# heracles-ec/heracles

Measured on AMD Instinct MI355X. Metric: map->Cl pairs/sec + mixing-matrix build sec, nside=4096 lmax=6144, higher is better.
Workload: dtype f64

## Files before the change

### heracles_amd/csrc/hx_analysis.hip

```cpp
#include <algorithm>
#include <cmath>
#include <cstdlib>
#include <cstring>

#include "hx_sht_common.h"

namespace hx {
using namespace hxfft;

constexpr int HALF_F = 1;
template <int SPIN>
struct LegCfg {
    static constexpr int NW = SPIN == 0 ? 16 : 8;
    static constexpr int NT = SPIN == 0 ? 1 : 2;
    static constexpr int NOP = SPIN == 0 ? 1 : 2;
    static constexpr int NPAR = (SPIN == 2 && HALF_F) ? 1 : 2;
};
int analysis_f_rows(int spin) { return spin == 0 ? LegCfg<0>::NPAR * LegCfg<0>::NOP : LegCfg<2>::NPAR * LegCfg<2>::NOP; }

struct LegParams {
    PlanDev P;
    const LegTask *__restrict__ tasks;
    const double *__restrict__ F;
    double *__restrict__ partial;
    int m0, ms;
    long long row0;
    int ng;
    int ncol;
    int pcol;
    const MTasks *__restrict__ of_m;
    const long long *__restrict__ arow;
    long long arow0;
    int add_all;
};

template <int SPIN>
__global__ __launch_bounds__(256) void k_fourier_combine(PlanDev P, const double2 *__restrict__ Y, int ncomp, int ng,
                                                         int ncol, int m0, int ms, const double *__restrict__ rw,
                                                         const LegTask *__restrict__ tasks, const MTasks *__restrict__ of_m,
                                                         double *__restrict__ F, int tile0)
{
    constexpr int NOP = LegCfg<SPIN>::NOP;
    __shared__ RingAtM ring_at_m[32];
    const int m = m0 + blockIdx.x * ms;
    const int ty = (int)blockIdx.y + tile0;
    const MTasks mt = of_m[m];
    if (mt.count == 0 || ty < tasks[mt.first].rb0) return;
    if (threadIdx.x < 32) ring_at_m[threadIdx.x] = ring_at_m_of(P, ty * 32 + threadIdx.x, m, rw);
    __syncthreads();
    const int rp = ty * 32 + (threadIdx.x >> 3);
    const int slot = threadIdx.x & 7;
    const bool live = rp < P.nrp;
    const RingAtM ram = ring_at_m[threadIdx.x >> 3];
    constexpr int NPAR = LegCfg<SPIN>::NPAR;
    double *row = F + (((long long)blockIdx.x * P.nrp_pad + rp) * NPAR) * NOP * ncol;
    for (int g = 0; g < ng; ++g) {
        if (SPIN == 0) {
            const int c = g * 8 + slot;
            if (g * NCOL + 2 * slot >= ncol) continue;
            double2 s = make_double2(0.0, 0.0), d = s;
            if (live && c < ncomp) {
                double2 fn, fs;
                ring_modes_ns(P, Y, c, rp, m, ram, fn, fs);
                s = cadd(fn, fs);
                d = csub(fn, fs);
            }
            *reinterpret_cast<double2 *>(row + g * NCOL + 2 * slot) = s;
            *reinterpret_cast<double2 *>(row + ncol + g * NCOL + 2 * slot) = d;
        } else {
            const int f = g * 4 + (slot >> 1), op = slot & 1;
            if (g * NCOL + 4 * (slot >> 1) >= ncol) continue;
            double4 o0 = make_double4(0.0, 0.0, 0.0, 0.0), o1 = o0;
            if (live && 2 * f + 1 < ncomp) {
                double2 qn, qs, un, us;
                ring_modes_ns(P, Y, 2 * f, rp, m, ram, qn, qs);
                ring_modes_ns(P, Y, 2 * f + 1, rp, m, ram, un, us);
                const double2 ppn = cscale(cadd(qn, mul_pi(un)), -0.5), pmn = cscale(csub(qn, mul_pi(un)), -0.5);
                const double2 pps = cscale(cadd(qs, mul_pi(us)), -0.5), pms = cscale(csub(qs, mul_pi(us)), -0.5);
                double4 x, y;
                if (op == 0) {
                    x = make_double4(ppn.x, ppn.y, ppn.y, -ppn.x);
                    y = make_double4(pms.x, pms.y, -pms.y, pms.x);
                } else {
                    x = make_double4(pmn.x, pmn.y, -pmn.y, pmn.x);
                    y = make_double4(pps.x, pps.y, pps.y, -pps.x);
                }
                o0 = make_double4(x.x + y.x, x.y + y.y, x.z + y.z, x.w + y.w);
                o1 = make_double4(x.x - y.x, x.y - y.y, x.z - y.z, x.w - y.w);
            }
            const int col = g * NCOL + 4 * (slot >> 1);
            *reinterpret_cast<double4 *>(row + (0 * NOP + op) * ncol + col) = o0;
            if (NPAR == 2) *reinterpret_cast<double4 *>(row + (1 * NOP + op) * ncol + col) = o1;
        }
    }
}

__device__ __host__ inline int tile_swz(int r) { return r & 15; }
__device__ __host__ inline int ringsel(int q, int k) { return (k & 1) * 16 + 2 * q + (k >> 1); }

template <int K>
__device__ inline int opaque(int v)
{
    asm("; opaque %1" : "+v"(v) : "n"(K));
    return v;
}

__device__ unsigned long long g_exec_flops[2];

template <int SPIN>
struct PipeCfg {
    static constexpr int NW = 4;
    static constexpr int RBS = SPIN == 0 ? 2 : 1;
    static constexpr int NCH = SPIN == 0 ? 2 : 1;
    static constexpr int NOP = SPIN == 0 ? 1 : 2;
};

__device__ __host__ inline int pipe_rho(int q, int k) { return 4 * q + k; }
__device__ __host__ inline int pipe_tile_idx(int c, int r) { return c * 32 + ((r ^ (c & 7)) * 2); }

constexpr int DUO_GAP = -1;
constexpr int DUO_PRIO = 1;
constexpr int DUO_ORDER = -1;
constexpr int DUO_SCALE_BITS2 = 100;
constexpr int DUO_SCALE_BITS0 = 300;

template <int K>
__device__ __forceinline__ double row_bcast(double v)
{
    double d;
    asm("v_mov_b64_dpp %0, %1 row_newbcast:%2 row_mask:0xf bank_mask:0xf" : "=v"(d) : "v"(v), "n"(K));
    return d;
}

template <int K>
__device__ __forceinline__ double row_bcast_fmac(double t, double p, double x)
{
    asm("v_fmac_f64_dpp %0, %1, %2 row_newbcast:%3 row_mask:0xf bank_mask:0xf" : "+v"(t) : "v"(p), "v"(x), "n"(K));
    return t;
}

template <int SPIN>
__device__ __forceinline__ void alm_rows_to_layout(const PlanDev &P, int m, bool any_task, const double *__restrict__ partial, long long r0, int ncol,
                                                   int ncomp, int ng, const double *__restrict__ fl, int add, double2 *__restrict__ alm,
                                                   long long alm_stride, const double *__restrict__ alphan, int tid, int nt)
{
    const int lmax = P.lmax;
    const int l0 = SPIN == 0 ? m : (m > 2 ? m : 2);
    const int nl = lmax - m + 1, nc = 8 * ng;
    constexpr int U = 8;
    for (int i0 = tid; i0 < nl * nc; i0 += nt * U) {
        double2 v[U];
        double al[U], f[U];
        long long dsti[U];
        bool on[U];
#pragma unroll
        for (int u = 0; u < U; ++u) {
            const int i = i0 + u * nt;
            const int l = m + i / nc, c = i % nc;
            on[u] = i < nl * nc && c < ncomp;
            v[u] = make_double2(0.0, 0.0);
            al[u] = 1.0;
            f[u] = 1.0;
            dsti[u] = 0;
            if (!on[u]) continue;
            dsti[u] = (long long)c * alm_stride + almidx(lmax, l, m);
            if (l >= l0 && any_task) {
                const double *prow = partial + (r0 + (l - l0)) * ncol + (c >> 3) * NCOL;
                v[u] = *reinterpret_cast<const double2 *>(prow + 2 * (c & 7));
                if (SPIN == 2 && alphan && ((l + m) & 1)) {
                    const int j = 2 * (c & 7);
                    v[u] = make_double2(prow[j ^ 3], prow[(j + 1) ^ 3]);
                }
                if (SPIN == 2 && HALF_F && ((l + m) & 1)) {
                    if (c & 1) v[u].y = -v[u].y;
                    else v[u].x = -v[u].x;
                }
                if (alphan) al[u] = alphan[almidx(lmax, l, m)];
                if (fl) f[u] = fl[l];
            }
        }
#pragma unroll
        for (int u = 0; u < U; ++u) {
            if (!on[u]) continue;
            double2 w = v[u];
            if (alphan) { w.x *= al[u]; w.y *= al[u]; }
            if (fl) { w.x *= f[u]; w.y *= f[u]; }
            double2 *dst = alm + dsti[u];
            if (add) { const double2 o = *dst; w.x += o.x; w.y += o.y; }
            *dst = w;
        }
    }
}

template <int SPIN, int NG, int NBX, int NSUB = 1>
__global__ __launch_bounds__(256, 2) void k_legendre_duo(LegParams A, const double2 *__restrict__ coefn)
{
    using C = PipeCfg<SPIN>;
    constexpr int NW = 4, NOP = C::NOP, NCH = C::NCH, NPAIR = 16;
    constexpr int NXA = NBX > 0 ? NBX : 1;
    constexpr int DQ0 = NG * 512, DSZ = NG * 512 + NBX * 128;
    constexpr bool HALFB = SPIN == 2;
    constexpr int SB = SPIN == 2 ? DUO_SCALE_BITS2 : DUO_SCALE_BITS0;
    constexpr int GAPN = DUO_GAP >= 0 ? DUO_GAP : ((SPIN == 2 && NG == 2 && NBX == 2) ? 5 : (SPIN == 2 && NG == 2 && NBX == 1) ? 6 : (SPIN == 2 && NG == 1 && NBX == 2) ? 0 : 4);
    constexpr int GORDER = DUO_ORDER >= 0 ? DUO_ORDER : ((SPIN == 2 && NG == 2 && NBX == 2) ? 2 : (SPIN == 0 && NG == 1 && NBX == 1) ? 1 : 0);
    constexpr int NPB = HALFB ? 1 : 2;
    constexpr int TW = NSUB * DSZ > 2048 ? NSUB * DSZ : 2048;
    static_assert(NG >= 1 && NG <= 2 && TW * NW * 8 <= 81920, "two work-groups per CU");
    static_assert(SPIN == 0 || HALF_F, "spin 2: the lambda- chain carries (-1)^(l + m) lambda- (one operand row, wave-uniform coefficients)");
    __shared__ double tile[NW][TW];
    __shared__ int lead_in[2][NW];
    const PlanDev &P = A.P;
    const int m = A.m0 + blockIdx.x * A.ms, lmax = P.lmax;
    const MTasks mt = A.of_m[m];
    const int l0 = SPIN == 0 ? m : (m > 2 ? m : 2);
    const int off = (l0 + m) & 1;
    const int nblk = (lmax - l0) / LBLK + 1;
    const long long orow = A.arow[m] - A.arow0;
    const double2 *__restrict__ cfm = coefn + almidx(lmax, 0, m) + l0 + (SPIN == 0 ? 0 : 1) + (threadIdx.x & 15);
    bool first_group = true;
    auto put = [&](double *p, double v) __attribute__((always_inline)) {
        if (first_group) *p = v;
        else __builtin_amdgcn_global_atomic_fadd_f64((__attribute__((address_space(1))) double *)p, v);
    };
    auto lds_barrier = []() __attribute__((always_inline)) {
        __builtin_amdgcn_s_waitcnt(0xc07f);
        __builtin_amdgcn_s_barrier();
    };
    int n_mf = 0, n_rec = 0;
    if (DUO_PRIO) __builtin_amdgcn_s_setprio(3);
    for (int ti = 0; ti < mt.count; ++ti) {
        const LegTask task = A.tasks[mt.first + ti];
        first_group = ti == 0 && !A.add_all;
        int tid = threadIdx.x;
        asm volatile("; ring group" : "+v"(tid));
        const int w = tid >> 6, lane = tid & 63;
        const int ai = lane & 15, ak = lane >> 4;
        if (ti) __syncthreads();

        const int rbi = SPIN == 0 ? 2 * w + (lane >> 5) : w;
        const int rpl = (task.rb0 + rbi) * RBLK + (lane & 31);
        const bool valid = rbi < task.nrb && rpl < P.nrp;
        const double x = valid ? P.z[rpl] : 0.0;
        const double xx = SPIN == 0 ? x * x : ((lane >> 5) ? -x : x);

        double fr[NPAIR][NPB][NG], frx[NPAIR][NPB][NXA];
#pragma unroll
        for (int sp = 0; sp < NPAIR; ++sp) {
// ... 323 lines not shown
        *dst = v;
    }
}

static int ring_mlim(int lmax, int spin, double sth, double cth)
{
    double ofs = lmax * 0.01;
    if (ofs < 100.) ofs = 100.;
    double b = -2 * spin * fabs(cth);
    double t1 = lmax * sth + ofs;
    double c = (double)spin * spin - t1 * t1;
    double discr = b * b - 4 * c;
    if (discr <= 0) return lmax;
    double res = (-b + sqrt(discr)) / 2.;
    if (res > lmax) res = lmax;
    return (int)(res + 0.5);
}

struct SweepShape {
    int ng, nbx, valu, ncol, oneset, duo;
};
static SweepShape sweep_shape(int spin, int nb)
{
    const int cols = 2 * nb;
    SweepShape sh = {0, 0, 0, 0, 0, 0};
    if (cols <= 8) { sh.valu = 1; return sh; }
    sh.duo = 1;
    sh.oneset = spin == 2;
    sh.ng = std::max(cols / NCOL, 1);
    const int rem = cols > NCOL ? cols % NCOL : 0;
    const int maxbx = spin == 2 ? 2 : (sh.ng == 1 ? 1 : 0);
    if (rem > 4 * maxbx) sh.ng += 1;
    else sh.nbx = (rem + 3) / 4;
    sh.ncol = NCOL * sh.ng + 4 * sh.nbx;
    return sh;
}
bool analysis_generic_spin(int spin)
{
    if (spin != 2) return spin != 0;
    const char *e = getenv("HX_SPIN_GENERIC");
    return e && atoi(e) != 0;
}
int analysis_max_comp(int spin) { return spin == 2 ? 8 * NGMAX + 4 : 8 * NGMAX; }

static double sweep_cost(int spin, int units)
{
    if (spin == 0) return units <= 4 ? 21.6 * units : (units <= 8 ? 84.1 : (units <= 10 ? 99.2 : 139.7));
    return units <= 2 ? 61.0 * units : (units <= 4 ? 164.5 : (units == 5 ? 194.1 : (units == 6 ? 222.0 : (units <= 8 ? 272.0 : (units == 9 ? 299.6 : 326.0)))));
}
int analysis_next_batch(int spin, int remaining)
{
    const int unit = spin == 0 ? 1 : 2, maxu = analysis_max_comp(spin) / unit;
    const int units = remaining / unit;
    if (units <= 0) return 0;
    std::vector<double> best(units + 1, 0.0);
    std::vector<int> first(units + 1, 0);
    for (int r = 1; r <= units; ++r) {
        best[r] = 1e300;
        for (int b = std::min(maxu, r); b >= 1; --b) {
            const double c = sweep_cost(spin, b) + best[r - b];
            if (c < best[r] - 1e-9) { best[r] = c; first[r] = b; }
        }
    }
    return unit * first[units];
}
int analysis_max_batch(int spin, int ncomp)
{
    int mx = 0;
    for (int left = ncomp; left > 0;) {
        const int nb = analysis_next_batch(spin, left);
        if (nb <= 0) break;
        mx = std::max(mx, nb);
        left -= nb;
    }
    return mx;
}

static int build_task_set(hx_plan *pl, int spin, int nw, hx_plan::TaskSet &ts);
int build_tasks(hx_plan *pl, int spin)
{
    return build_task_set(pl, spin, spin == 0 ? LegCfg<0>::NW : LegCfg<2>::NW, pl->ts[spin ? 1 : 0]);
}
static int build_task_set(hx_plan *pl, int spin, int nw, hx_plan::TaskSet &ts)
{
    if (ts.built) return HX_OK;
    const int lmax = pl->lmax;
    const int nrb = (pl->nrp + RBLK - 1) / RBLK;
    ts.tasks.clear();
    ts.of_m.assign(lmax + 1, MTasks{0, 0});
    ts.rows_before_m.assign(lmax + 2, 0);
    ts.arow.assign(lmax + 2, 0);
    long long rows = 0, arows = 0;
    std::vector<int> mlim(pl->nrp);
    for (int rp = 0; rp < pl->nrp; ++rp) mlim[rp] = ring_mlim(lmax, spin, pl->h_sth[rp], pl->h_z[rp]);
    for (int m = 0; m <= lmax; ++m) {
        ts.rows_before_m[m] = rows;
        ts.arow[m] = arows;
        const int l0 = std::max(m, spin);
        if (l0 <= lmax) arows += (long long)LBLK * ((lmax - l0) / LBLK + 1);
        ts.of_m[m].first = (int)ts.tasks.size();
        if (l0 <= lmax) {
            int first = (int)(std::lower_bound(mlim.begin(), mlim.end(), m) - mlim.begin());
            if (first >= pl->nrp) first = pl->nrp - 1;
            for (int rb = first / RBLK; rb < nrb; rb += nw) {
                LegTask t;
                t.m = m; t.rb0 = rb; t.nrb = std::min(nw, nrb - rb); t.pad = 0; t.pout = rows;
                rows += (long long)LBLK * ((lmax - l0) / LBLK + 1);
                ts.tasks.push_back(t);
            }
        }
        ts.of_m[m].count = (int)ts.tasks.size() - ts.of_m[m].first;
    }
    ts.rows_before_m[lmax + 1] = rows;
    ts.arow[lmax + 1] = arows;
    HX_TRY(upload(ts.d_tasks, ts.tasks));
    HX_TRY(upload(ts.d_of_m, ts.of_m));
    HX_TRY(upload(ts.d_arow, ts.arow));
    ts.built = true;
    return HX_OK;
}

static bool duo_shape(const SweepShape &sh) { return sh.duo != 0; }
static int sweep_pcol(const SweepShape &sh) { return sh.ncol > 2 * NCOL ? (sh.ncol + 15) / 16 * 16 : sh.ncol; }

template <int SPIN>
static int launch_duo(const SweepShape &sh, dim3 pgrid, hipStream_t st, const LegParams &A, const double2 *cn)
{
    const dim3 db(256);
    const int key = sh.ng * 10 + sh.nbx;
    if (key == 10) hipLaunchKernelGGL((k_legendre_duo<SPIN, 1, 0, 2>), pgrid, db, 0, st, A, cn);
    else if (key == 11) hipLaunchKernelGGL((k_legendre_duo<SPIN, 1, 1, 2>), pgrid, db, 0, st, A, cn);
    else if (key == 20 && SPIN == 2) hipLaunchKernelGGL((k_legendre_duo<2, 2, 0, 2>), pgrid, db, 0, st, A, cn);
    else if (key == 12 && SPIN == 2) hipLaunchKernelGGL((k_legendre_duo<2, 1, 2, 2>), pgrid, db, 0, st, A, cn);
    else if (key == 21 && SPIN == 2) hipLaunchKernelGGL((k_legendre_duo<2, 2, 1, 2>), pgrid, db, 0, st, A, cn);
    else if (key == 20) hipLaunchKernelGGL((k_legendre_duo<SPIN, 2, 0>), pgrid, db, 0, st, A, cn);
    else if (key == 22 && SPIN == 2) hipLaunchKernelGGL((k_legendre_duo<2, 2, 2>), pgrid, db, 0, st, A, cn);
    else return fail(HX_ERR_ARG, "legendre analysis: no two-group kernel for %d groups + %d blocks", sh.ng, sh.nbx);
    return HX_OK;
}

template <int SPIN>
static int launch_chunk(hx_plan *pl, hx_plan::TaskSet &ts, int m0, int m1, int nb, const SweepShape &sh, const double *d_rw,
                        const double *d_fl, int add, double2 *d_alms)
{
    const int ng = sh.ng + (sh.nbx > 0 ? 1 : 0), ncol = sh.ncol;
    const int pcol = sweep_pcol(sh);
    hipStream_t st = rt().stream;
    PlanDev P = pl->dev();
    const int t0 = ts.of_m[m0].first;
    const int t1 = ts.of_m[m1 - 1].first + ts.of_m[m1 - 1].count;
    const int ms = std::max(pl->m_step, 1), nm = (m1 - m0 + ms - 1) / ms;
    {
        ProfScope ps("fourier_combine");
        dim3 grid(nm, pl->nrp_pad / 32);
        hipLaunchKernelGGL(k_fourier_combine<SPIN>, grid, dim3(256), 0, st, P, pl->Y.as<double2>(), nb, ng, ncol, m0, ms, d_rw,
                           ts.d_tasks.as<LegTask>(), ts.d_of_m.as<MTasks>(), pl->F.as<double>(), 0);
    }
    if (t1 > t0) {
        ProfScope ps("legendre_analysis");
        ProfScope ps2(SPIN == 0 ? "legendre_analysis_s0" : "legendre_analysis_s2");
        LegParams A;
        A.P = P; A.tasks = ts.d_tasks.as<LegTask>() + t0; A.F = pl->F.as<double>(); A.partial = pl->partial.as<double>();
        A.m0 = m0; A.ms = ms; A.row0 = ts.rows_before_m[m0]; A.ng = ng; A.ncol = ncol; A.pcol = pcol;
        A.of_m = ts.d_of_m.as<MTasks>(); A.arow = ts.d_arow.as<long long>(); A.arow0 = ts.arow[m0]; A.add_all = 0;
        A.tasks = ts.d_tasks.as<LegTask>();
        const double2 *cn = SPIN == 0 ? pl->cn0.as<double2>() : pl->cn2.as<double2>();
        HX_TRY(launch_duo<SPIN>(sh, dim3((unsigned)nm), st, A, cn));
    }
    {
        ProfScope ps("alm_reduce");
        hipLaunchKernelGGL(k_alm_reduce<SPIN>, dim3(nm), dim3(256), 0, st, P, ts.d_tasks.as<LegTask>(), ts.d_of_m.as<MTasks>(),
                           pl->partial.as<double>(), ts.arow[m0], m0, ms, nb, ng, pcol, d_fl, add, d_alms, pl->nlm, ts.d_arow.as<long long>(),
                           SPIN == 0 ? pl->al0.as<double>() : pl->al2.as<double>());
    }
    HX_HIP(hipGetLastError());
    return HX_OK;
}

static bool valu_batch(int spin, int nb) { return sweep_shape(spin, nb).valu != 0; }

int valu_tasks(hx_plan *pl, int spin, hx_plan::TaskSet **out, int blocks, bool generic)
{
    if (generic) {
        hx_plan::SpinSet *set = nullptr;
        HX_TRY(ensure_rec_s(pl, spin, &set));
        HX_TRY(build_task_set(pl, spin, valu_task_blocks(spin), set->ts));
        *out = &set->ts;
        return HX_OK;
    }
    if (spin) HX_TRY(ensure_rec2(pl));
    if (blocks <= 0) blocks = valu_task_blocks(spin);
    if (blocks != valu_task_blocks(spin) && blocks != 8) return fail(HX_ERR_ARG, "valu_tasks: %d ring blocks per task", blocks);
    hx_plan::TaskSet &ts = blocks == 8 && blocks != valu_task_blocks(spin) ? (spin ? pl->ts[6] : pl->ts[7]) : (spin ? pl->ts[4] : pl->ts[5]);
    HX_TRY(build_task_set(pl, spin, blocks, ts));
    *out = &ts;
    return HX_OK;
}

int synth_duo_tasks(hx_plan *pl, int spin, hx_plan::TaskSet **out)
{
    if (spin) HX_TRY(ensure_rec2(pl));
    hx_plan::TaskSet &ts = spin ? pl->ts[3] : pl->ts[2];
    HX_TRY(build_task_set(pl, spin, PipeCfg<2>::NW * (spin ? PipeCfg<2>::RBS : PipeCfg<0>::RBS), ts));
    DevBuf &lim = spin ? pl->syn_mlim2 : pl->syn_mlim0;
    if (!lim.p) {
        std::vector<int> h(pl->nrp_pad, -1);
        for (int rp = 0; rp < pl->nrp; ++rp) {
            const int last = std::min(rp / RBLK * RBLK + RBLK - 1, pl->nrp - 1);
            h[rp] = std::min(pl->lmax, ring_mlim(pl->lmax, spin, pl->h_sth[last], pl->h_z[last]));
        }
        HX_TRY(upload(lim, h));
    }
    *out = &ts;
    return HX_OK;
}

static int analysis_batch_valu(hx_plan *pl, int spin, int nb, const double *d_maps, double2 *d_alms, const double *d_rw,
                               const double *d_pw, const double *d_fl, int add, bool generic = false)
{
    hx_plan::TaskSet *tsp = nullptr;
    HX_TRY(valu_tasks(pl, spin, &tsp, 0, generic));
    hx_plan::TaskSet &ts = *tsp;
    if (pl->hsrc == nullptr && pl->nssrc == nullptr) {
        HX_TRY(pl->Y.alloc(sizeof(double2) * (size_t)pl->ny * nb));
        HX_TRY(launch_ring_subdft_maps(pl, nb, d_maps, d_pw, pl->Y.as<double2>()));
    }
    double budget = 80e9;
    if (scratch_budget_bytes() > 0.0) budget = scratch_budget_bytes();
    else {
        size_t fr = 0, tot = 0;
        if (hipMemGetInfo(&fr, &tot) == hipSuccess) budget = std::min(budget, 0.5 * (double)(fr + pl->F.bytes + pl->partial.bytes));
        budget = std::max(budget, 2e9);
    }
    const int lmax = pl->lmax, pcol = valu_partial_cols(spin), unit = spin ? 2 : 1;
    const double f_per_m = (double)pl->nrp_pad * valu_operand_doubles(spin) * sizeof(double);
    const std::vector<long long> &prow = ts.rows_before_m;
    std::vector<std::pair<int, int>> chunks;
    size_t maxF = 16, maxP = 16;
    const int m_end = pl->m_hi < 0 ? lmax + 1 : std::min(pl->m_hi, lmax + 1), ms = std::max(pl->m_step, 1);
    for (int m0 = std::max(pl->m_lo, 0); m0 < m_end;) {
        int last = m0;
        while (last + ms < m_end) {
            const double bytes = f_per_m * ((last + ms - m0) / ms + 1) + (double)(prow[last + ms + 1] - prow[m0]) * pcol * sizeof(double);
            if (bytes > budget) break;
            last += ms;
        }
        const int m1 = last + 1;
        chunks.emplace_back(m0, m1);
        maxF = std::max(maxF, (size_t)(f_per_m * ((m1 - m0 + ms - 1) / ms)));
        maxP = std::max(maxP, (size_t)(prow[m1] - prow[m0]) * pcol * sizeof(double));
        m0 = last + ms;
    }
    HX_TRY(pl->F.alloc(maxF));
    HX_TRY(pl->partial.alloc(maxP));
    pl->last_chunks = (int)chunks.size();
    PlanDev P = pl->dev();
    for (int c0 = 0; c0 < nb; c0 += unit)
        for (auto &ch : chunks) {
            const int m0 = ch.first, m1 = ch.second, nm = (m1 - m0 + ms - 1) / ms;
            HX_TRY(launch_valu_chunk(pl, spin, ts, m0, m1, c0, d_rw, generic));
            ProfScope ps("alm_reduce");
            if (generic)
                hipLaunchKernelGGL(k_alm_reduce_spin, dim3(nm), dim3(256), 0, rt().stream, lmax, spin, ts.d_tasks.as<LegTask>(), ts.d_of_m.as<MTasks>(),
                                   pl->partial.as<double>(), ts.rows_before_m[m0], m0, ms, d_fl, add, d_alms + (size_t)c0 * pl->nlm, pl->nlm);
            else if (spin == 0)
                hipLaunchKernelGGL(k_alm_reduce<0>, dim3(nm), dim3(256), 0, rt().stream, P, ts.d_tasks.as<LegTask>(), ts.d_of_m.as<MTasks>(),
                                   pl->partial.as<double>(), ts.rows_before_m[m0], m0, ms, 1, 1, pcol, d_fl, add, d_alms + (size_t)c0 * pl->nlm, pl->nlm, nullptr, nullptr);
            else
                hipLaunchKernelGGL(k_alm_reduce<2>, dim3(nm), dim3(256), 0, rt().stream, P, ts.d_tasks.as<LegTask>(), ts.d_of_m.as<MTasks>(),
                                   pl->partial.as<double>(), ts.rows_before_m[m0], m0, ms, 2, 1, pcol, d_fl, add, d_alms + (size_t)c0 * pl->nlm, pl->nlm, nullptr, nullptr);
            HX_HIP(hipGetLastError());
        }
    return HX_OK;
}

int analysis_batch(hx_plan *pl, int spin, int nb, const double *d_maps, double2 *d_alms, const double *d_rw,
                   const double *d_pw, const double *d_fl, int add)
{
    const bool generic = plan_generic_spin(pl, spin);
    if (generic || (spin != 0 && spin != 2)) {
        if (!generic) return fail(HX_ERR_UNSUPPORTED, "spin-%d maps not yet supported", spin);
        if (spin < 0 || nb < 2 || (nb & 1)) return fail(HX_ERR_ARG, "analysis_batch: %d components of spin %d", nb, spin);
        if (spin > pl->lmax) {
            if (!add) HX_HIP(hipMemsetAsync(d_alms, 0, sizeof(double2) * (size_t)pl->nlm * nb, rt().stream));
            return HX_OK;
        }
        return analysis_batch_valu(pl, spin, nb, d_maps, d_alms, d_rw, d_pw, d_fl, add, true);
    }
    if (valu_batch(spin, nb)) return analysis_batch_valu(pl, spin, nb, d_maps, d_alms, d_rw, d_pw, d_fl, add);
    const int sidx = spin ? 1 : 0;
    HX_TRY(build_tasks(pl, spin));
    if (spin) HX_TRY(ensure_rec2(pl));
    const SweepShape sh = sweep_shape(spin, nb);
    const bool one_set = sh.oneset || duo_shape(sh);
    if (one_set) HX_TRY(build_task_set(pl, spin, PipeCfg<2>::NW * (spin ? PipeCfg<2>::RBS : PipeCfg<0>::RBS), spin ? pl->ts[3] : pl->ts[2]));
    hx_plan::TaskSet &ts = one_set ? (spin ? pl->ts[3] : pl->ts[2]) : pl->ts[sidx];
    const int ncol = sh.ncol;
    if (pl->hsrc == nullptr && pl->nssrc == nullptr) {
        HX_TRY(pl->Y.alloc(sizeof(double2) * (size_t)pl->ny * nb));
        HX_TRY(launch_ring_subdft_maps(pl, nb, d_maps, d_pw, pl->Y.as<double2>()));
    }

    double budget = 80e9;
    if (scratch_budget_bytes() > 0.0) budget = scratch_budget_bytes();
    else {
        size_t fr = 0, tot = 0;
        if (hipMemGetInfo(&fr, &tot) == hipSuccess)
            budget = std::min(budget, 0.5 * (double)(fr + pl->F.bytes + pl->partial.bytes));
        budget = std::max(budget, 2e9);
    }
    const double f_per_m = (double)pl->nrp_pad * analysis_f_rows(spin) * ncol * sizeof(double);
    const int lmax = pl->lmax;
    const std::vector<long long> &prow = ts.arow;
    const int pcol = sweep_pcol(sh);
    std::vector<std::pair<int, int>> chunks;
    size_t maxF = 16, maxP = 16;
    const int m_end = pl->m_hi < 0 ? lmax + 1 : std::min(pl->m_hi, lmax + 1), ms = std::max(pl->m_step, 1);
    for (int m0 = std::max(pl->m_lo, 0); m0 < m_end;) {
        int last = m0;
        while (last + ms < m_end) {
            const double bytes = f_per_m * ((last + ms - m0) / ms + 1) + (double)(prow[last + ms + 1] - prow[m0]) * pcol * sizeof(double);
            if (bytes > budget) break;
            last += ms;
        }
        const int m1 = last + 1;
        chunks.emplace_back(m0, m1);
        maxF = std::max(maxF, (size_t)(f_per_m * ((m1 - m0 + ms - 1) / ms)));
        maxP = std::max(maxP, (size_t)(prow[m1] - prow[m0]) * pcol * sizeof(double));
        m0 = last + ms;
    }
    HX_TRY(pl->F.alloc(maxF));
    HX_TRY(pl->partial.alloc(maxP));
    pl->last_chunks = (int)chunks.size();
    for (auto &ch : chunks) {
        if (spin == 0)
            HX_TRY(launch_chunk<0>(pl, ts, ch.first, ch.second, nb, sh, d_rw, d_fl, add, d_alms));
        else
            HX_TRY(launch_chunk<2>(pl, ts, ch.first, ch.second, nb, sh, d_rw, d_fl, add, d_alms));
    }
    return HX_OK;
}

static hx_plan::TaskSet &stream_tasks(hx_plan *pl, int spin) { return spin ? pl->ts[3] : pl->ts[2]; }

bool analysis_can_stream(hx_plan *pl, int spin, int nb)
{
    if (!pl || pl->nside < 1 || pl->hsrc || pl->nssrc || pl->m_lo != 0 || pl->m_hi >= 0 || pl->m_step > 1) return false;
    if (nb < 1 || nb > analysis_max_comp(spin)) return false;
    const SweepShape sh = sweep_shape(spin, nb);
    if (!duo_shape(sh) || sh.valu) return false;
    const double f_bytes = (double)pl->nrp_pad * analysis_f_rows(spin) * sh.ncol * sizeof(double) * (pl->lmax + 1.0);
    const double p_bytes = 0.5 * (pl->lmax + 1.0) * (pl->lmax + 2.0 + LBLK) * sweep_pcol(sh) * sizeof(double);
    double budget = 80e9;
    if (scratch_budget_bytes() > 0.0) budget = scratch_budget_bytes();
    if (f_bytes + p_bytes > budget) return false;
    size_t fr = 0, tot = 0;
    if (hipMemGetInfo(&fr, &tot) != hipSuccess) {
        (void)hipGetLastError();
        return false;
    }
    const double y_bytes = (double)pl->ny * nb * sizeof(double2), stage_bytes = 2.0 * nb * (double)pl->npix * sizeof(double);
    const double held = (double)pl->F.bytes + (double)pl->partial.bytes + (double)pl->Y.bytes + (double)pl->stage[0].bytes + (double)pl->stage[1].bytes +
                        (double)pl->stage[2].bytes;
    return f_bytes + p_bytes + y_bytes + stage_bytes <= 0.95 * ((double)fr + held);
}

int analysis_stream_plan(hx_plan *pl, int spin, int nb, int nslab, StreamSweep &s)
{
    if (!analysis_can_stream(pl, spin, nb)) return fail(HX_ERR_ARG, "analysis_stream_plan: not a streamable sweep");
    if (spin) HX_TRY(ensure_rec2(pl));
    HX_TRY(build_task_set(pl, spin, PipeCfg<2>::NW * (spin ? PipeCfg<2>::RBS : PipeCfg<0>::RBS), stream_tasks(pl, spin)));
    hx_plan::TaskSet &ts = stream_tasks(pl, spin);
    const SweepShape sh = sweep_shape(spin, nb);
    s.pl = pl; s.spin = spin; s.nb = nb;
    const int nrb = (pl->nrp + RBLK - 1) / RBLK;
    std::vector<double> cum(nrb + 1, 0.0);
    for (int rb = 0; rb < nrb; ++rb) {
        double px = 0.0;
        for (int rp = rb * RBLK; rp < std::min((rb + 1) * RBLK, pl->nrp); ++rp) px += (rp == pl->nrp - 1 ? 4.0 : 8.0) * pl->h_nsub[rp];
        cum[rb + 1] = cum[rb] + px;
    }
    nslab = std::max(1, std::min(nslab, nrb));
    s.rp_edge.assign(1, 0);
    for (int k = 1; k < nslab; ++k) {
        const int rb = (int)(std::lower_bound(cum.begin(), cum.end(), cum[nrb] * k / nslab) - cum.begin());
        if (rb * RBLK > s.rp_edge.back() && rb < nrb) s.rp_edge.push_back(rb * RBLK);
    }
    s.rp_edge.push_back(nrb * RBLK);
    s.nslab = (int)s.rp_edge.size() - 1;
    const int lmax = pl->lmax;
    std::vector<MTasks> tab((size_t)s.nslab * (lmax + 1), MTasks{0, 0});
    for (int m = 0; m <= lmax; ++m) {
        const MTasks mt = ts.of_m[m];
        int t = mt.first;
        for (int k = 0; k < s.nslab; ++k) {
            const int rb_hi = s.rp_edge[k + 1] / RBLK;
            MTasks &o = tab[(size_t)k * (lmax + 1) + m];
            o.first = t;
            while (t < mt.first + mt.count && ts.tasks[t].rb0 + ts.tasks[t].nrb <= rb_hi) ++t;
            o.count = t - o.first;
        }
        if (t != mt.first + mt.count) return fail(HX_ERR_ARG, "analysis_stream_plan: ring groups of m = %d left over", m);
    }
    HX_TRY(upload(s.d_of_m, tab));
    HX_TRY(pl->Y.alloc(sizeof(double2) * (size_t)pl->ny * nb));
    HX_TRY(pl->F.alloc((size_t)pl->nrp_pad * analysis_f_rows(spin) * sh.ncol * sizeof(double) * (size_t)(lmax + 1)));
    HX_TRY(pl->partial.alloc((size_t)ts.arow[lmax + 1] * sweep_pcol(sh) * sizeof(double)));
    return HX_OK;
}

int analysis_stream_start(StreamSweep &s)
{
    hx_plan *pl = s.pl;
    const SweepShape sh = sweep_shape(s.spin, s.nb);
    HX_HIP(hipMemsetAsync(pl->partial.p, 0, (size_t)stream_tasks(pl, s.spin).arow[pl->lmax + 1] * sweep_pcol(sh) * sizeof(double), rt().stream));
    pl->last_chunks = 1;
    return HX_OK;
}

template <int SPIN>
static int stream_slab(StreamSweep &s, int k)
{
    hx_plan *pl = s.pl;
    hx_plan::TaskSet &ts = stream_tasks(pl, SPIN);
    const SweepShape sh = sweep_shape(SPIN, s.nb);
    const int ng = sh.ng + (sh.nbx > 0 ? 1 : 0), lmax = pl->lmax, nm = lmax + 1;
    const int rp_lo = s.rp_edge[k], rp_hi = s.rp_edge[k + 1];
    hipStream_t st = rt().stream;
    PlanDev P = pl->dev();
    HX_TRY(launch_ring_subdft_maps(pl, s.nb, s.d_maps, s.d_pw, pl->Y.as<double2>(), rp_lo, std::min(rp_hi, pl->nrp)));
    {
        ProfScope ps("fourier_combine");
        const int tile_hi = k + 1 == s.nslab ? pl->nrp_pad / 32 : rp_hi / 32;
        dim3 grid(nm, tile_hi - rp_lo / 32);
        hipLaunchKernelGGL(k_fourier_combine<SPIN>, grid, dim3(256), 0, st, P, pl->Y.as<double2>(), s.nb, ng, sh.ncol, 0, 1, s.d_rw,
                           ts.d_tasks.as<LegTask>(), ts.d_of_m.as<MTasks>(), pl->F.as<double>(), rp_lo / 32);
    }
    {
        ProfScope ps("legendre_analysis");
        ProfScope ps2(SPIN == 0 ? "legendre_analysis_s0" : "legendre_analysis_s2");
        LegParams A;
        A.P = P; A.tasks = ts.d_tasks.as<LegTask>(); A.F = pl->F.as<double>(); A.partial = pl->partial.as<double>();
        A.m0 = 0; A.ms = 1; A.row0 = 0; A.ng = ng; A.ncol = sh.ncol; A.pcol = sweep_pcol(sh);
        A.of_m = s.d_of_m.as<MTasks>() + (size_t)k * (lmax + 1); A.arow = ts.d_arow.as<long long>(); A.arow0 = 0; A.add_all = 1;
        HX_TRY(launch_duo<SPIN>(sh, dim3((unsigned)nm), st, A, SPIN == 0 ? pl->cn0.as<double2>() : pl->cn2.as<double2>()));
    }
    HX_HIP(hipGetLastError());
    return HX_OK;
}

int analysis_stream_slab(StreamSweep &s, int k)
{
    if (k < 0 || k >= s.nslab) return fail(HX_ERR_ARG, "analysis_stream_slab: slab %d of %d", k, s.nslab);
    return s.spin == 0 ? stream_slab<0>(s, k) : stream_slab<2>(s, k);
}

int analysis_stream_end(StreamSweep &s)
{
    hx_plan *pl = s.pl;
    hx_plan::TaskSet &ts = stream_tasks(pl, s.spin);
    const SweepShape sh = sweep_shape(s.spin, s.nb);
    const int ng = sh.ng + (sh.nbx > 0 ? 1 : 0), nm = pl->lmax + 1, pcol = sweep_pcol(sh);
    PlanDev P = pl->dev();
    ProfScope ps("alm_reduce");
    if (s.spin == 0)
        hipLaunchKernelGGL(k_alm_reduce<0>, dim3(nm), dim3(256), 0, rt().stream, P, ts.d_tasks.as<LegTask>(), ts.d_of_m.as<MTasks>(), pl->partial.as<double>(),
                           0LL, 0, 1, s.nb, ng, pcol, s.d_fl, 0, s.d_alms, pl->nlm, ts.d_arow.as<long long>(), pl->al0.as<double>());
    else
        hipLaunchKernelGGL(k_alm_reduce<2>, dim3(nm), dim3(256), 0, rt().stream, P, ts.d_tasks.as<LegTask>(), ts.d_of_m.as<MTasks>(), pl->partial.as<double>(),
                           0LL, 0, 1, s.nb, ng, pcol, s.d_fl, 0, s.d_alms, pl->nlm, ts.d_arow.as<long long>(), pl->al2.as<double>());
    HX_HIP(hipGetLastError());
    return HX_OK;
}

}

extern "C" int hx_plan_mfma_flops(hx_plan *pl, int spin, int ncomp, double *flops)
{
    using namespace hx;
    if (!pl || !flops || ncomp < 1 || (spin != 0 && spin != 2)) return fail(HX_ERR_ARG, "hx_plan_mfma_flops: bad arguments");
    HX_TRY(ensure_ready());
    HX_TRY(build_tasks(pl, spin));
    const hx_plan::TaskSet &ts = pl->ts[spin ? 1 : 0];
    const int nop = spin ? 2 : 1, l0min = spin ? 2 : 0;
    double wave_blocks = 0.0;
    for (const LegTask &t : ts.tasks) {
        const int l0 = std::max(t.m, l0min);
        wave_blocks += (double)t.nrb * ((pl->lmax - l0) / LBLK + 1);
    }
    double per_wave_block = 0.0;
    for (int c0 = 0, nb = 0; c0 < ncomp; c0 += nb) {
        nb = analysis_next_batch(spin, ncomp - c0);
        const SweepShape sh = sweep_shape(spin, nb);
        per_wave_block += 16.0 * nop * (sh.ng * 2048.0 + sh.nbx * 512.0);
    }
    *flops = wave_blocks * per_wave_block;
    return HX_OK;
}

extern "C" int hx_executed_flops(double *out2, int reset)
{
    using namespace hx;
    if (!out2) return fail(HX_ERR_ARG, "hx_executed_flops: null output");
    HX_TRY(ensure_ready());
    HX_HIP(hipStreamSynchronize(rt().stream));
    unsigned long long v[2] = {0, 0}, w = 0;
    HX_HIP(hipMemcpyFromSymbol(v, HIP_SYMBOL(g_exec_flops), sizeof(v)));
    HX_TRY(valu_exec_flops(&w, reset != 0));
    if (reset) {
        const unsigned long long z[2] = {0, 0};
        HX_HIP(hipMemcpyToSymbol(HIP_SYMBOL(g_exec_flops), z, sizeof(z)));
    }
    out2[0] = (double)v[0];
    out2[1] = (double)v[1] + (double)w;
    return HX_OK;
}

extern "C" int hx_plan_executed_flops(hx_plan *pl, int spin, int ncomp, double *out2)
{
    using namespace hx;
    if (!out2) return fail(HX_ERR_ARG, "hx_plan_executed_flops: null output");
    HX_TRY(hx_plan_mfma_flops(pl, spin, ncomp, &out2[0]));
    const hx_plan::TaskSet &ts = pl->ts[spin ? 1 : 0];
    const int nop = spin ? 2 : 1, l0min = spin ? 2 : 0;
    double wave_blocks = 0.0;
    for (const LegTask &t : ts.tasks) {
        const int l0 = std::max(t.m, l0min);
        wave_blocks += (double)t.nrb * ((pl->lmax - l0) / LBLK + 1);
    }
    int sweeps = 0;
    for (int c0 = 0, nb = 0; c0 < ncomp; c0 += nb, ++sweeps) nb = analysis_next_batch(spin, ncomp - c0);
    out2[1] = wave_blocks * sweeps * (double)RBLK * LBLK * nop * 4.0;
    return HX_OK;
}
```

### heracles_amd/csrc/hx_sht_common.h

```cpp
#pragma once
#include <map>
#include <vector>

#include "hx_common.h"
#include "hx_fft_core.h"

namespace hx {

typedef double double4_t __attribute__((ext_vector_type(4)));

constexpr int LBLK = 32;
constexpr int NCOL = 16;
constexpr int TABLE_PAD = 512;
constexpr int NGMAX = 2;
constexpr int RBLK = 32;
constexpr double SC_BIG = 0x1p+300, SC_SMALL = 0x1p-300;
constexpr int SPIN_ANY = -1;

struct LegTask {
    int m;
    int rb0;
    int nrb;
    int pad;
    long long pout;
};

struct MTasks {
    int first, count;
};

struct alignas(16) RingDesc {
    long long sN, sS, bhat_off;
    int n, rp;
};
struct PlanDev {
    int nside, lmax, nrp, nrp_pad, twN;
    long long npix, ny;
    const double *z, *omz, *sth, *rwdef;
    const int *nsub, *shifted;
    const long long *startN, *startS, *bhat_off;
    const double2 *tw, *bhat;
    const double *mfac, *kfac2;
    const double2 *rec0;
    const double4 *rec2;
    double wnorm;
    const double2 *hsrc;
    long long hsrc_stride;
    int hN;
    const double4 *const *nssrc;
    int ns_m0, ns_ms;
};

__host__ __device__ inline long long almidx(int lmax, int l, int m)
{
    return (long long)m * (2 * lmax + 1 - m) / 2 + l;
}

__device__ inline double2 expipi(double x)
{
    double s, c;
    sincospi(x, &s, &c);
    return make_double2(c, s);
}

struct SVal {
    double v;
    int e;
};

__device__ inline void snorm_small(SVal &s)
{
    if (s.v != 0.0)
        while (fabs(s.v) < SC_SMALL) {
            s.v *= SC_BIG;
            s.e -= 1;
        }
}

template <int SB>
__device__ inline void sval_rebase(double &v, int &e)
{
    static_assert(300 % SB == 0, "the step must divide 300");
    if (SB != 300) {
        constexpr double big = SB == 100 ? 0x1p+100 : SB == 150 ? 0x1p+150 : SB == 75 ? 0x1p+75 : SB == 60 ? 0x1p+60 : 0x1p+50;
        static_assert(SB == 300 || SB == 100 || SB == 150 || SB == 75 || SB == 60 || SB == 50, "unsupported step");
        e *= 300 / SB;
        if (v != 0.0)
            while (fabs(v) < 1.0 / big) {
                v *= big;
                e -= 1;
            }
    }
}

__device__ inline SVal spow(double x, int n)
{
    SVal r = {1.0, 0}, b = {x, 0};
    while (n) {
        if (n & 1) {
            r.v *= b.v;
            r.e += b.e;
            snorm_small(r);
        }
        n >>= 1;
        if (n) {
            b.v *= b.v;
            b.e *= 2;
            snorm_small(b);
        }
    }
    return r;
}

__device__ inline double sval_true(double v, int e)
{
    return e == 0 ? v : (e == -1 ? v * SC_SMALL : 0.0);
}

__device__ inline void spin2_seeds(int m, double sth, double omx, double kfac2m, SVal &sp, SVal &sm)
{
    const int l0 = m > 2 ? m : 2;
    const double opx = 2.0 - omx;
    const double nrm = sqrt((2.0 * l0 + 1.0) / (4.0 * M_PI));
    if (m == 0) {
        const double d = 0.61237243569579452455 * sth * sth;
        sp.v = sm.v = nrm * d; sp.e = sm.e = 0;
    } else if (m == 1) {
        sp.v = nrm * (-0.5 * omx * sth); sp.e = 0;
        sm.v = nrm * (0.5 * opx * sth);  sm.e = 0;
    } else {
        SVal b = spow(sth, m - 2);
        b.v *= kfac2m * nrm * ((m & 1) ? -1.0 : 1.0);
        sp.v = b.v * (0.25 * omx * omx); sp.e = b.e;
        sm.v = b.v * (0.25 * opx * opx); sm.e = b.e;
    }
    snorm_small(sp);
    snorm_small(sm);
}

__device__ inline void spin_seeds(int s, int m, double sth, double omx, double kfsm, SVal &sp, SVal &sm)
{
    const double opx = 2.0 - omx;
    SVal b = spow(sth, m >= s ? m - s : s - m);
    b.v *= kfsm;
    const int n = m >= s ? s : m;
    const SVal ps = spow(0.5 * omx, n), pc = spow(0.5 * opx, n);
    sp.v = b.v * ps.v; sp.e = b.e + ps.e;
    sm.v = b.v * pc.v; sm.e = b.e + pc.e;
    if (m < s) {
        if (m & 1) sp.v = -sp.v;
        if (s & 1) sm.v = -sm.v;
    }
    snorm_small(sp);
    snorm_small(sm);
}

#ifdef __HIPCC__
using namespace hxfft;
struct RingAtM {
    double2 ph;
    long long i0, i1;
    int hasS;
};

__device__ inline void ring_modes_ns(const PlanDev &P, const double2 *__restrict__ Y, int c, int rp, int m,
                                     const RingAtM &r, double2 &FN, double2 &FS, int s = 0)
{
    if (P.nssrc) {
        const double4 v = P.nssrc[c][(long long)((m - P.ns_m0) / P.ns_ms) * P.nrp_pad + rp];
        FN = make_double2(v.x, v.y);
        FS = make_double2(v.z, v.w);
        return;
    }
    if (P.hsrc) {
        const double w = r.ph.x;
        const double2 *h = P.hsrc + (long long)c * P.hsrc_stride + (long long)m * P.hN;
        const double sg = ((m + s) & 1) ? -w : w;
        const double2 a = h[rp], b = h[P.hN - 1 - rp], cN = h[P.hN / 2 - 1 - rp], d = h[P.hN / 2 + rp];
        FN = make_double2(w * a.x + sg * b.x, w * a.y + sg * b.y);
        FS = make_double2(w * cN.x + sg * d.x, w * cN.y + sg * d.y);
        return;
    }
    const double2 *Yc = Y + (long long)c * P.ny;
    const double2 a = Yc[r.i0], b = cconj(Yc[r.i1]);
    const double2 xn = cscale(cadd(a, b), 0.5);
    const double2 xs = mul_mi(cscale(csub(a, b), 0.5));
    FN = cmul(xn, r.ph);
    FS = r.hasS ? cmul(xs, r.ph) : make_double2(0.0, 0.0);
}

__device__ inline RingAtM ring_at_m_of(const PlanDev &P, int r, int m, const double *__restrict__ rw)
{
    RingAtM q;
    const bool live = r < P.nrp;
    const double w = live ? (rw ? rw[r] : 1.0) * P.wnorm : 0.0;
    q.ph = make_double2(w, 0.0);
    q.i0 = q.i1 = 0;
    q.hasS = 0;
    if (live && !P.hsrc) {
        const int n = P.nsub[r], nphi = 4 * n;
        const int mm = m % nphi, mc = (nphi - mm) % nphi;
        q.i0 = P.startN[r] + (long long)(mm & 3) * n + (mm >> 2);
        q.i1 = P.startN[r] + (long long)(mc & 3) * n + (mc >> 2);
        if (P.shifted[r]) q.ph = cscale(expipi(-(double)(m % (2 * nphi)) / (double)nphi), w);
        q.hasS = P.startS[r] >= 0;
    }
    return q;
}

template <class TW>
__device__ __forceinline__ void lds_fft_pass_dif(double2 *buf, int M, int K, int h, int gt, int gn, TW tw, int twN)
{
    switch (K) {
    case 4:
_Pragma("unroll 1")
        for (int i = gt; i < (M >> 4); i += gn) dif_pass_butterfly<4>(buf, i, h, tw, twN); break;
    case 3:
_Pragma("unroll 1")
        for (int i = gt; i < (M >> 3); i += gn) dif_pass_butterfly<3>(buf, i, h, tw, twN); break;
    case 2:
_Pragma("unroll 1")
        for (int i = gt; i < (M >> 2); i += gn) dif_pass_butterfly<2>(buf, i, h, tw, twN); break;
    default: for (int i = gt; i < (M >> 1); i += gn) dif_pass_butterfly<1>(buf, i, h, tw, twN); break;
    }
}
template <class TW>
__device__ __forceinline__ void lds_fft_pass_dit_inv(double2 *buf, int M, int K, int h, int gt, int gn, TW tw, int twN)
{
    switch (K) {
    case 4:
_Pragma("unroll 1")
        for (int i = gt; i < (M >> 4); i += gn) dit_inv_pass_butterfly<4>(buf, i, h, tw, twN); break;
    case 3:
_Pragma("unroll 1")
        for (int i = gt; i < (M >> 3); i += gn) dit_inv_pass_butterfly<3>(buf, i, h, tw, twN); break;
    case 2:
_Pragma("unroll 1")
        for (int i = gt; i < (M >> 2); i += gn) dit_inv_pass_butterfly<2>(buf, i, h, tw, twN); break;
    default: for (int i = gt; i < (M >> 1); i += gn) dit_inv_pass_butterfly<1>(buf, i, h, tw, twN); break;
    }
}
template <class TW>
__device__ __forceinline__ void lds_fft_dif(double2 *buf, int M, TW tw, int twN, int gt, int gn, bool skip_last = false)
{
    const int p = ilog2(M), np = fft_sched_np(p);
    int h = M;
    for (int a = 0; a < np - (skip_last ? 1 : 0); ++a) {
        const int K = fft_sched_k(p, a);
        h >>= K;
        lds_fft_pass_dif(buf, M, K, h, gt, gn, tw, twN);
        __syncthreads();
    }
}
template <class TW>
__device__ __forceinline__ void lds_fft_dit_inv(double2 *buf, int M, TW tw, int twN, int gt, int gn, bool skip_first = false)
{
    const int p = ilog2(M), np = fft_sched_np(p);
    int h = 1;
    for (int a = np - 1; a >= 0; --a) {
        const int K = fft_sched_k(p, a);
        if (!(skip_first && a == np - 1)) {
            lds_fft_pass_dit_inv(buf, M, K, h, gt, gn, tw, twN);
            __syncthreads();
        }
        h <<= K;
    }
}
template <class TW>
__device__ __forceinline__ void lds_fft_dif(double2 *buf, int M, TW tw, int twN) { lds_fft_dif(buf, M, tw, twN, (int)threadIdx.x, (int)blockDim.x); }
template <class TW>
__device__ __forceinline__ void lds_fft_dit_inv(double2 *buf, int M, TW tw, int twN) { lds_fft_dit_inv(buf, M, tw, twN, (int)threadIdx.x, (int)blockDim.x); }

constexpr int TW_HI_MAX = 128;
__device__ inline TwFactored load_tw_factored(double2 *hi, double2 *lo, const double2 *__restrict__ tw, int twN)
{
    for (int i = threadIdx.x; i < (twN >= 128 ? twN / 128 : 1); i += blockDim.x) hi[i] = tw[i * 64];
    for (int i = threadIdx.x; i < 64; i += blockDim.x) lo[i] = tw[i];
    TwFactored f;
    f.hi = hi;
    f.lo = lo;
    return f;
}

#endif

template <class T>
inline int upload(DevBuf &b, const std::vector<T> &v)
{
    HX_TRY(b.alloc(sizeof(T) * (v.size() > 0 ? v.size() : 1)));
    if (!v.empty()) HX_HIP(hipMemcpy(b.p, v.data(), sizeof(T) * v.size(), hipMemcpyHostToDevice));
    return HX_OK;
}

}

struct hx_plan {
    int nside = 0, lmax = 0, max_comp = 0;
    int nrp = 0, nrp_pad = 0, twN = 1;
    int fft_cap = 8192;
    int last_chunks = 0;
    int eqN = 0;
    double wnorm = 0.0;
    const double2 *hsrc = nullptr;
    long long hsrc_stride = 0;
    const double4 *const *nssrc = nullptr;
    int ns_m0 = 0;
    int m_lo = 0, m_hi = -1, m_step = 1;
    long long npix = 0, ny = 0, nlm = 0;
    size_t lds_fft = 0;
    hx::DevBuf z, omz, sth, rwdef, nsub, shifted, startN, startS, bhat_off, tw, bhat, mfac, kfac2, rec0, rec2, cn0, al0, cn2, al2;
    std::vector<double> h_sth, h_z;
    std::vector<int> h_nsub;
    std::vector<long long> h_startN, h_startS;
    struct TaskSet {
        bool built = false;
        std::vector<hx::LegTask> tasks;
        std::vector<hx::MTasks> of_m;
        std::vector<long long> rows_before_m;
        std::vector<long long> arow;
        hx::DevBuf d_tasks, d_of_m, d_arow;
    } ts[8];
    struct SpinSet {
        hx::DevBuf cn, al, kf;
        TaskSet ts;
    };
    std::map<int, SpinSet> spin_sets;
    struct FftClass { int M, first, count, big; };
    std::vector<FftClass> fft_classes;
    hx::DevBuf fft_rp_list;
    hx::DevBuf fft_desc;
    std::vector<int> h_fft_rp_list;
    hx::DevBuf Y, F, partial, d_dbg, resid_maps, pw_sym;
    hx::DevBuf syn_mlim0, syn_mlim2;
    hx::DevBuf syn_tab, syn_boff0, syn_boff2;
    const double *pw_checked = nullptr;
    int pw_mode = 0;
    static constexpr int NSTAGE = 3;
    hx::DevBuf stage[NSTAGE];
    hipEvent_t stage_done[NSTAGE] = {nullptr, nullptr, nullptr};
    static constexpr int NUNIT_EV = 4;
    hipEvent_t unit_up[NUNIT_EV] = {nullptr, nullptr, nullptr, nullptr};
// ... 50 lines not shown
```

Before: 422.8.

## Tile Fourier-combine over order×ring-pair blocks with shuffle-transposed gathers

Adds a tiled fourier_combine kernel in which each block covers 32 orders by 8 ring pairs. Ring metadata (phase, gather indices, flags) is computed once per (order, ring) into shared memory. Y gathers are issued with lanes mapped so that consecutive orders hit adjacent bins, then redistributed to the output layout via warp shuffles, and blocks are swizzled across the grid. The aim is to turn scattered per-component gathers into coalesced loads and to skip tiles with no active tasks. The old kernel is kept as a fallback for the hsrc/nssrc paths, m_step>1, or too many groups, at the cost of extra shuffles and shared-memory staging.

```diff
diff --git a/heracles_amd/csrc/hx_analysis.hip b/heracles_amd/csrc/hx_analysis.hip
--- a/heracles_amd/csrc/hx_analysis.hip
+++ b/heracles_amd/csrc/hx_analysis.hip
@@ -93,6 +93,150 @@
             if (NPAR == 2) *reinterpret_cast<double4 *>(row + (1 * NOP + op) * ncol + col) = o1;
         }
     }
+}
+
+constexpr int FC_TM = 32;
+constexpr int FC_RP = 8;
+constexpr int FC_NG = NGMAX + 1;
+constexpr int FC_U = 4;
+static_assert(FC_RP % FC_U == 0 && FC_TM * FC_RP == 256, "a thread per (order, ring pair); whole rounds of ring pairs");
+
+__device__ __forceinline__ double2 lane_from(const double2 v, int src) { return make_double2(__shfl(v.x, src), __shfl(v.y, src)); }
+
+template <int SPIN>
+__global__ __launch_bounds__(256) void k_fourier_combine_tiled(PlanDev P, const double2 *__restrict__ Y, int ncomp, int ng, int ncol, int m0, int nm,
+                                                               const double *__restrict__ rw, const LegTask *__restrict__ tasks,
+                                                               const MTasks *__restrict__ of_m, double *__restrict__ F, int rp_lo, int rp_hi,
+                                                               int ntile_m, int nwork)
+{
+    constexpr int NOP = LegCfg<SPIN>::NOP, NPAR = LegCfg<SPIN>::NPAR;
+    constexpr int FL_ON = 1, FL_S = 2, FL_LIVE = 4;
+    __shared__ double2 sh_ph[FC_TM * FC_RP];
+    __shared__ long long sh_i0[FC_TM * FC_RP], sh_i1[FC_TM * FC_RP];
+    __shared__ int sh_flag[FC_TM * FC_RP];
+    __shared__ int any;
+    const int tid = threadIdx.x;
+    const int w = ((int)blockIdx.x & 7) * ((int)gridDim.x >> 3) + ((int)blockIdx.x >> 3);
+    if (w >= nwork) return;
+    const int Mt = ((m0 >> 5) + w % ntile_m) * FC_TM;
+    const int rp0 = rp_lo + (w / ntile_m) * FC_RP;
+    if (tid == 0) any = 0;
+    __syncthreads();
+    {
+        const int m = Mt + (tid & 31), rp = rp0 + (tid >> 5);
+        const bool in = m >= m0 && m < m0 + nm && rp < rp_hi;
+        RingAtM q = ring_at_m_of(P, in ? rp : P.nrp, in ? m : 0, rw);
+        int fl = 0;
+        if (in) {
+            const MTasks mt = of_m[m];
+            if (mt.count != 0 && (rp >> 5) >= tasks[mt.first].rb0) {
+                fl = FL_ON | (q.hasS ? FL_S : 0) | (rp < P.nrp ? FL_LIVE : 0);
+                any = 1;
+            }
+        }
+        sh_ph[tid] = q.ph;
+        sh_i0[tid] = q.i0;
+        sh_i1[tid] = q.i1;
+        sh_flag[tid] = fl;
+    }
+    __syncthreads();
+    if (!any) return;
+
+    const int lane = tid & 63, j = tid >> 6;
+    const int kL = lane & 7, sL = lane >> 3;
+    const int kC = lane >> 3, sC = lane & 7;
+    const int m = Mt + 4 * kC + j;
+    for (int rpl0 = 0; rpl0 < FC_RP; rpl0 += FC_U) {
+        double2 a[FC_U][FC_NG], b[FC_U][FC_NG];
+#pragma unroll
+        for (int u = 0; u < FC_U; ++u) {
+            const int miL = (rpl0 + u) * FC_TM + 4 * kL + j;
+            const int flL = sh_flag[miL];
+            const bool ld = (flL & (FL_ON | FL_LIVE)) == (FL_ON | FL_LIVE);
+            const double2 *ya = Y + sh_i0[miL], *yb = Y + sh_i1[miL];
+#pragma unroll
+            for (int g = 0; g < FC_NG; ++g) {
+                const int c = g * 8 + sL;
+                const bool on = g < ng && ld && c < ncomp;
+                a[u][g] = on ? ya[(long long)c * P.ny] : make_double2(0.0, 0.0);
+                b[u][g] = on ? yb[(long long)c * P.ny] : make_double2(0.0, 0.0);
+            }
+        }
+#pragma unroll
+        for (int u = 0; u < FC_U; ++u) {
+            const int rpl = rpl0 + u;
+            const int miC = rpl * FC_TM + 4 * kC + j;
+            const int flC = sh_flag[miC];
+            if (!__any(flC & FL_ON)) continue;
+            const int rp = rp0 + rpl;
+            const bool on = flC & FL_ON, live = flC & FL_LIVE;
+            RingAtM ram;
+            ram.ph = sh_ph[miC];
+            ram.hasS = (flC & FL_S) ? 1 : 0;
+            double *row = F + (((long long)(m - m0) * P.nrp_pad + rp) * NPAR) * NOP * ncol;
+#pragma unroll
+            for (int g = 0; g < FC_NG; ++g) {
+                if (SPIN == 0) {
+                    const double2 za = lane_from(a[u][g], sC * 8 + kC), zb = lane_from(b[u][g], sC * 8 + kC);
+                    const int c = g * 8 + sC;
+                    if (g < ng && on && g * NCOL + 2 * sC < ncol) {
+                        double2 s = make_double2(0.0, 0.0), d = s;
+                        if (live && c < ncomp) {
+                            double2 fn, fs;
+                            ring_modes_of_bins(za, zb, ram, fn, fs);
+                            s = cadd(fn, fs);
+                            d = csub(fn, fs);
+                        }
+                        *reinterpret_cast<double2 *>(row + g * NCOL + 2 * sC) = s;
+                        *reinterpret_cast<double2 *>(row + ncol + g * NCOL + 2 * sC) = d;
+                    }
+                } else {
+                    const int lq = (sC & 6) * 8 + kC, lu = lq + 8;
+                    const double2 qa = lane_from(a[u][g], lq), qb = lane_from(b[u][g], lq), ua = lane_from(a[u][g], lu), ub = lane_from(b[u][g], lu);
+                    const int f = g * 4 + (sC >> 1), op = sC & 1;
+                    if (g < ng && on && g * NCOL + 4 * (sC >> 1) < ncol) {
+                        double4 o0 = make_double4(0.0, 0.0, 0.0, 0.0), o1 = o0;
+                        if (live && 2 * f + 1 < ncomp) {
+                            double2 qn, qs, un, us;
+                            ring_modes_of_bins(qa, qb, ram, qn, qs);
+                            ring_modes_of_bins(ua, ub, ram, un, us);
+                            const double2 ppn = cscale(cadd(qn, mul_pi(un)), -0.5), pmn = cscale(csub(qn, mul_pi(un)), -0.5);
+                            const double2 pps = cscale(cadd(qs, mul_pi(us)), -0.5), pms = cscale(csub(qs, mul_pi(us)), -0.5);
+                            double4 x, y;
+                            if (op == 0) {
+                                x = make_double4(ppn.x, ppn.y, ppn.y, -ppn.x);
+                                y = make_double4(pms.x, pms.y, -pms.y, pms.x);
+                            } else {
+                                x = make_double4(pmn.x, pmn.y, -pmn.y, pmn.x);
+                                y = make_double4(pps.x, pps.y, pps.y, -pps.x);
+                            }
+                            o0 = make_double4(x.x + y.x, x.y + y.y, x.z + y.z, x.w + y.w);
+                            o1 = make_double4(x.x - y.x, x.y - y.y, x.z - y.z, x.w - y.w);
+                        }
+                        const int col = g * NCOL + 4 * (sC >> 1);
+                        *reinterpret_cast<double4 *>(row + (0 * NOP + op) * ncol + col) = o0;
+                        if (NPAR == 2) *reinterpret_cast<double4 *>(row + (1 * NOP + op) * ncol + col) = o1;
+                    }
+                }
+            }
+        }
+    }
+}
+
+template <int SPIN>
+static void launch_fourier_combine(const PlanDev &P, const double2 *Y, int nb, int ng, int ncol, int m0, int ms, int nm, const double *d_rw,
+                                   const LegTask *tasks, const MTasks *of_m, double *F, int tile0, int tile_hi, hipStream_t st)
+{
+    if (P.hsrc || P.nssrc || ms != 1 || ng > FC_NG) {
+        dim3 grid(nm, tile_hi - tile0);
+        hipLaunchKernelGGL(k_fourier_combine<SPIN>, grid, dim3(256), 0, st, P, Y, nb, ng, ncol, m0, ms, d_rw, tasks, of_m, F, tile0);
+        return;
+    }
+    const int rp_lo = tile0 * 32, rp_hi = tile_hi * 32;
+    const int ntile_m = ((m0 + nm - 1) >> 5) - (m0 >> 5) + 1;
+    const int nwork = ntile_m * ((rp_hi - rp_lo) / FC_RP);
+    hipLaunchKernelGGL(k_fourier_combine_tiled<SPIN>, dim3((unsigned)((nwork + 7) / 8 * 8)), dim3(256), 0, st, P, Y, nb, ng, ncol, m0, nm, d_rw,
+                       tasks, of_m, F, rp_lo, rp_hi, ntile_m, nwork);
 }
 
 __device__ __host__ inline int tile_swz(int r) { return r & 15; }
@@ -722,9 +866,8 @@
     const int ms = std::max(pl->m_step, 1), nm = (m1 - m0 + ms - 1) / ms;
     {
         ProfScope ps("fourier_combine");
-        dim3 grid(nm, pl->nrp_pad / 32);
-        hipLaunchKernelGGL(k_fourier_combine<SPIN>, grid, dim3(256), 0, st, P, pl->Y.as<double2>(), nb, ng, ncol, m0, ms, d_rw,
-                           ts.d_tasks.as<LegTask>(), ts.d_of_m.as<MTasks>(), pl->F.as<double>(), 0);
+        launch_fourier_combine<SPIN>(P, pl->Y.as<double2>(), nb, ng, ncol, m0, ms, nm, d_rw, ts.d_tasks.as<LegTask>(), ts.d_of_m.as<MTasks>(),
+                                     pl->F.as<double>(), 0, pl->nrp_pad / 32, st);
     }
     if (t1 > t0) {
         ProfScope ps("legendre_analysis");
@@ -1002,9 +1145,8 @@
     {
         ProfScope ps("fourier_combine");
         const int tile_hi = k + 1 == s.nslab ? pl->nrp_pad / 32 : rp_hi / 32;
-        dim3 grid(nm, tile_hi - rp_lo / 32);
-        hipLaunchKernelGGL(k_fourier_combine<SPIN>, grid, dim3(256), 0, st, P, pl->Y.as<double2>(), s.nb, ng, sh.ncol, 0, 1, s.d_rw,
-                           ts.d_tasks.as<LegTask>(), ts.d_of_m.as<MTasks>(), pl->F.as<double>(), rp_lo / 32);
+        launch_fourier_combine<SPIN>(P, pl->Y.as<double2>(), s.nb, ng, sh.ncol, 0, 1, nm, s.d_rw, ts.d_tasks.as<LegTask>(), ts.d_of_m.as<MTasks>(),
+                                     pl->F.as<double>(), rp_lo / 32, tile_hi, st);
     }
     {
         ProfScope ps("legendre_analysis");
diff --git a/heracles_amd/csrc/hx_sht_common.h b/heracles_amd/csrc/hx_sht_common.h
--- a/heracles_amd/csrc/hx_sht_common.h
+++ b/heracles_amd/csrc/hx_sht_common.h
@@ -163,6 +163,15 @@
     int hasS;
 };
 
+__device__ __forceinline__ void ring_modes_of_bins(const double2 a, const double2 braw, const RingAtM &r, double2 &FN, double2 &FS)
+{
+    const double2 b = cconj(braw);
+    const double2 xn = cscale(cadd(a, b), 0.5);
+    const double2 xs = mul_mi(cscale(csub(a, b), 0.5));
+    FN = cmul(xn, r.ph);
+    FS = r.hasS ? cmul(xs, r.ph) : make_double2(0.0, 0.0);
+}
+
 __device__ inline void ring_modes_ns(const PlanDev &P, const double2 *__restrict__ Y, int c, int rp, int m,
                                      const RingAtM &r, double2 &FN, double2 &FS, int s = 0)
 {
@@ -182,11 +191,7 @@
         return;
     }
     const double2 *Yc = Y + (long long)c * P.ny;
-    const double2 a = Yc[r.i0], b = cconj(Yc[r.i1]);
-    const double2 xn = cscale(cadd(a, b), 0.5);
-    const double2 xs = mul_mi(cscale(csub(a, b), 0.5));
-    FN = cmul(xn, r.ph);
-    FS = r.hasS ? cmul(xs, r.ph) : make_double2(0.0, 0.0);
+    ring_modes_of_bins(Yc[r.i0], Yc[r.i1], r, FN, FS);
 }
 
 __device__ inline RingAtM ring_at_m_of(const PlanDev &P, int r, int m, const double *__restrict__ rw)
```

After: 426.2, median of 6. Within noise of the previous version (+0.8%).
